# faasm/faabric

Hardware: NVIDIA H100
Metric: mpi_allreduce_resnet50_grads_algbw_GBps (higher is better)
Workload: dtype int32

## Files before the change

### csrc/kernels/coll_move_bulk.cu

```cuda
#include "coll_move.cuh"

namespace fb {

namespace {
constexpr uint32_t BULK_TILE = 32 * 1024;
constexpr int BULK_STAGES = 4;

__device__ __forceinline__ uint32_t smemPtr(const void* p)
{
    return (uint32_t)__cvta_generic_to_shared(p);
}

__device__ __forceinline__ void mbarInit(uint64_t* bar, uint32_t count)
{
    asm volatile("mbarrier.init.shared::cta.b64 [%0], %1;" ::"r"(smemPtr(bar)), "r"(count) : "memory");
}

__device__ __forceinline__ void mbarExpectTx(uint64_t* bar, uint32_t bytes)
{
    asm volatile("mbarrier.arrive.expect_tx.shared::cta.b64 _, [%0], %1;" ::"r"(smemPtr(bar)), "r"(bytes) : "memory");
}

__device__ __forceinline__ void mbarWait(uint64_t* bar, uint32_t parity)
{
    uint32_t done = 0;
    while (!done) {
        asm volatile("{\n\t"
                     ".reg .pred p;\n\t"
                     "mbarrier.try_wait.parity.shared::cta.b64 p, [%1], %2;\n\t"
                     "selp.u32 %0, 1, 0, p;\n\t"
                     "}"
                     : "=r"(done)
                     : "r"(smemPtr(bar)), "r"(parity)
                     : "memory");
    }
}

__device__ __forceinline__ void bulkLoad(void* smemDst, const void* gsrc, uint32_t bytes, uint64_t* bar)
{
    asm volatile("cp.async.bulk.shared::cluster.global.mbarrier::complete_tx::bytes [%0], [%1], %2, [%3];" ::"r"(
                   smemPtr(smemDst)),
                 "l"(gsrc),
                 "r"(bytes),
                 "r"(smemPtr(bar))
                 : "memory");
}

__device__ __forceinline__ void bulkStore(void* gdst, const void* smemSrc, uint32_t bytes)
{
    asm volatile("cp.async.bulk.global.shared::cta.bulk_group [%0], [%1], %2;" ::"l"(gdst), "r"(smemPtr(smemSrc)), "r"(bytes)
                 : "memory");
    asm volatile("cp.async.bulk.commit_group;" ::: "memory");
}

__device__ __forceinline__ void bulkWaitRead0()
{
    asm volatile("cp.async.bulk.wait_group.read 0;" ::: "memory");
}

__device__ __forceinline__ void bulkWaitAll()
{
    asm volatile("cp.async.bulk.wait_group 0;" ::: "memory");
}

__device__ __forceinline__ void fenceProxyAsync()
{
    asm volatile("fence.proxy.async;" ::: "memory");
}

struct Piece
{
    const uint8_t* src;
    uint8_t* dst;
};
}

__global__ void __launch_bounds__(128, 1) moveBulkKernel(const MoveArgs a)
{
    extern __shared__ __align__(128) uint8_t smem[];
    __shared__ __align__(8) uint64_t full[BULK_STAGES];

    BlockBarrier bar;
    bar.load(a.comm);
    bool ok = true;
    if (!a.noSync) {
        ok = bar.sync(a.comm);
    }
    const int rank = a.comm.rank;
    const int n = a.comm.nranks;

    if (threadIdx.x == 0) {
        for (int s = 0; s < BULK_STAGES; s++) {
            mbarInit(&full[s], 1);
        }
        asm volatile("fence.mbarrier_init.release.cluster;" ::: "memory");
        fenceProxyAsync();
    }
    __syncthreads();

    if (ok && threadIdx.x == 0) {
        int nPieces = 0;
        int firstPeer = 0;
        if (a.mode == MOVE_ALLGATHER || a.mode == MOVE_ALLTOALL || (a.mode == MOVE_GATHER && rank == a.root)) {
            nPieces = n;
            firstPeer = rank;
        } else if (a.mode == MOVE_SCATTER || (a.mode == MOVE_BCAST && rank != a.root)) {
            nPieces = 1;
        }
        const uint64_t srcExtra = (a.mode == MOVE_ALLTOALL) ? (uint64_t)rank * a.srcStride : 0;
        const uint64_t tilesPerPiece = (a.chunkBytes + BULK_TILE - 1) / BULK_TILE;
        const uint64_t totalTiles = (uint64_t)nPieces * tilesPerPiece;

        auto tileSrcDst = [&](uint64_t t, const uint8_t*& src, uint8_t*& dst, uint32_t& bytes) {
            const int q = (int)(t % (uint64_t)max(nPieces, 1));
            const uint64_t k = t / (uint64_t)max(nPieces, 1);
            const uint64_t off = k * BULK_TILE;
            bytes = (uint32_t)min((uint64_t)BULK_TILE, a.chunkBytes - off);
            if (a.mode == MOVE_SCATTER) {
                src = a.comm.heap[a.root] + a.sendOff + (uint64_t)rank * a.srcStride + off;
                dst = a.recvLocal + off;
            } else if (a.mode == MOVE_BCAST) {
                src = a.comm.heap[a.root] + a.sendOff + off;
                dst = a.recvLocal + off;
            } else {
                const int p = (firstPeer + q) % n;
                src = a.comm.heap[p] + a.sendOff + srcExtra + off;
                dst = a.recvLocal + (uint64_t)p * a.dstStride + off;
            }
        };

        const uint64_t first = blockIdx.x;
        const uint64_t step = gridDim.x;
        uint64_t nMine = first < totalTiles ? (totalTiles - first + step - 1) / step : 0;

        for (uint64_t j = 0; j < nMine && j < (uint64_t)BULK_STAGES; j++) {
            const uint8_t* src;
            uint8_t* dst;
            uint32_t bytes;
            tileSrcDst(first + j * step, src, dst, bytes);
            mbarExpectTx(&full[j], bytes);
            bulkLoad(smem + j * BULK_TILE, src, bytes, &full[j]);
        }
        for (uint64_t j = 0; j < nMine; j++) {
            const int s = (int)(j % BULK_STAGES);
            const uint32_t parity = (uint32_t)((j / BULK_STAGES) & 1);
            const uint8_t* src;
            uint8_t* dst;
            uint32_t bytes;
            tileSrcDst(first + j * step, src, dst, bytes);
            mbarWait(&full[s], parity);
            bulkStore(dst, smem + s * BULK_TILE, bytes);
// ... 76 lines not shown
```

### csrc/kernels/coll_reduce.cuh

```cuda
#pragma once

#include "fb_prims.cuh"
#include "launch_api.h"

namespace fb {

template<typename VR, int NR>
__device__ __forceinline__ Vec16 gatherReduce(const ReduceArgs& a,
                                              uint64_t byteOff)
{
    if constexpr (NR > 0) {
        Vec16 v[NR];
#pragma unroll
        for (int p = 0; p < NR; p++) {
            v[p] = ldVecStream(a.comm.heap[p] + a.sendOff + byteOff);
        }
        Vec16 acc = v[0];
#pragma unroll
        for (int p = 1; p < NR; p++) {
            acc = VR::apply(acc, v[p]);
        }
        return acc;
    } else {
        Vec16 acc = ldVecStream(a.comm.heap[0] + a.sendOff + byteOff);
// ... 310 lines not shown
        memcpy(&out, &v, 4);
    } else if constexpr (sizeof(E) == 8) {
        uint64_t v = *reinterpret_cast<const volatile uint64_t*>(p);
        memcpy(&out, &v, 8);
    } else {
        Vec16 v = ldVec(p);
        memcpy(&out, &v, 16);
    }
    return out;
}

template<typename E>
__device__ __forceinline__ void stElemGlobal(uint8_t* p, const E& in)
{
    if constexpr (sizeof(E) == 1) {
        uint8_t v;
        memcpy(&v, &in, 1);
        *reinterpret_cast<volatile uint8_t*>(p) = v;
    } else if constexpr (sizeof(E) == 2) {
        uint16_t v;
        memcpy(&v, &in, 2);
        *reinterpret_cast<volatile uint16_t*>(p) = v;
    } else if constexpr (sizeof(E) == 4) {
        uint32_t v;
        memcpy(&v, &in, 4);
        *reinterpret_cast<volatile uint32_t*>(p) = v;
    } else if constexpr (sizeof(E) == 8) {
        uint64_t v;
        memcpy(&v, &in, 8);
        *reinterpret_cast<volatile uint64_t*>(p) = v;
    } else {
        Vec16 v;
        memcpy(&v, &in, 16);
        stVec(p, v);
    }
}

template<typename VR>
__device__ __forceinline__ void groupTail(const FbCommDev& c,
                                          const GroupSeg& sg,
                                          int n)
{
    using Elem = typename VR::Elem;
    constexpr uint32_t EB = VR::ELEM_BYTES;
    const uint64_t base = (uint64_t)sg.nVec * 16;
    for (uint32_t e = 0; e + EB <= sg.tailBytes; e += EB) {
        Elem acc = ldElemGlobal<Elem>(c.heap[0] + sg.sendOff + base + e);
        for (int p = 1; p < n; p++) {
            Elem v = ldElemGlobal<Elem>(c.heap[p] + sg.sendOff + base + e);
            acc = VR::combine(acc, v);
        }
        for (int p = 0; p < n; p++) {
            stElemGlobal<Elem>(c.heap[p] + sg.recvOff + base + e, acc);
        }
    }
}

template<typename VR, int NR>
__global__ void __launch_bounds__(512, 1) groupAllReduceKernel(
  const GroupArgs a)
{
    extern __shared__ __align__(16) uint8_t sGroupRaw[];
    GroupSeg* sSegs = reinterpret_cast<GroupSeg*>(sGroupRaw);
    const FbCommDev& c = a.comm;
    const int n = (NR > 0) ? NR : c.nranks;
    {
        const Vec16* src = reinterpret_cast<const Vec16*>(a.segs);
        Vec16* dst = reinterpret_cast<Vec16*>(sGroupRaw);
        for (uint32_t i = threadIdx.x; i < a.nSegs * 2; i += blockDim.x) {
            dst[i] = src[i];
        }
    }
    BlockBarrier bar;
    bar.epoch = 0;
    bool ok = true;
    if (!a.noSync) {
        bar.load(c);
        ok = bar.sync(c);
    } else {
        __syncthreads();
    }

    if (ok && a.nSegs > 0) {
        constexpr int UNROLL = (NR == 8) ? 2 : (NR == 1 ? 8 : 4);
        constexpr uint32_t CHUNK = 32u * UNROLL;
        const uint32_t lane = threadIdx.x & 31;
        const uint32_t warpsPerCta = blockDim.x >> 5;
        const uint32_t warpStride = gridDim.x * warpsPerCta;
        int cur = 0;
        for (uint32_t ch = blockIdx.x * warpsPerCta + (threadIdx.x >> 5);
             ch < a.totalChunks;
             ch += warpStride) {
            if (!(sSegs[cur].chunk0 <= ch &&
                  (cur + 1 == (int)a.nSegs || ch < sSegs[cur + 1].chunk0))) {
                int lo = 0;
                int hi = (int)a.nSegs - 1;
                while (lo < hi) {
                    int mid = (lo + hi + 1) >> 1;
                    if (sSegs[mid].chunk0 <= ch) {
                        lo = mid;
                    } else {
                        hi = mid - 1;
                    }
                }
                cur = lo;
            }
            const GroupSeg sg = sSegs[cur];
            const uint32_t v0 = (ch - sg.chunk0) * CHUNK;
            const uint64_t sOff = sg.sendOff + (uint64_t)v0 * 16;
            const uint64_t rOff = sg.recvOff + (uint64_t)v0 * 16;
            const uint32_t rem = sg.nVec > v0 ? sg.nVec - v0 : 0;
            if (rem >= CHUNK) {
                Vec16 acc[UNROLL];
                if constexpr (NR > 0) {
                    Vec16 v[UNROLL][NR];
#pragma unroll
                    for (int u = 0; u < UNROLL; u++) {
#pragma unroll
                        for (int p = 0; p < NR; p++) {
                            v[u][p] = ldVecStream(c.heap[p] + sOff +
                                                  (uint64_t)(u * 32 + lane) * 16);
                        }
                    }
#pragma unroll
                    for (int u = 0; u < UNROLL; u++) {
                        acc[u] = v[u][0];
#pragma unroll
                        for (int p = 1; p < NR; p++) {
                            acc[u] = VR::apply(acc[u], v[u][p]);
                        }
                    }
#pragma unroll
                    for (int u = 0; u < UNROLL; u++) {
#pragma unroll
                        for (int p = 0; p < NR; p++) {
                            stVec(c.heap[p] + rOff + (uint64_t)(u * 32 + lane) * 16,
                                  acc[u]);
                        }
                    }
                } else {
#pragma unroll
                    for (int u = 0; u < UNROLL; u++) {
                        acc[u] = ldVecStream(c.heap[0] + sOff +
                                             (uint64_t)(u * 32 + lane) * 16);
                    }
                    for (int p = 1; p < n; p++) {
                        Vec16 v[UNROLL];
#pragma unroll
                        for (int u = 0; u < UNROLL; u++) {
                            v[u] = ldVecStream(c.heap[p] + sOff +
                                               (uint64_t)(u * 32 + lane) * 16);
                        }
#pragma unroll
                        for (int u = 0; u < UNROLL; u++) {
                            acc[u] = VR::apply(acc[u], v[u]);
                        }
                    }
                    for (int p = 0; p < n; p++) {
#pragma unroll
                        for (int u = 0; u < UNROLL; u++) {
                            stVec(c.heap[p] + rOff + (uint64_t)(u * 32 + lane) * 16,
                                  acc[u]);
                        }
                    }
                }
            } else {
#pragma unroll
                for (int u = 0; u < UNROLL; u++) {
                    const uint32_t i = (uint32_t)u * 32 + lane;
                    if (i < rem) {
                        Vec16 acc = ldVecStream(c.heap[0] + sOff + (uint64_t)i * 16);
                        for (int p = 1; p < n; p++) {
                            Vec16 v = ldVecStream(c.heap[p] + sOff + (uint64_t)i * 16);
                            acc = VR::apply(acc, v);
                        }
                        for (int p = 0; p < n; p++) {
                            stVec(c.heap[p] + rOff + (uint64_t)i * 16, acc);
                        }
                    }
                }
                if (sg.tailBytes != 0 && lane == 0 && v0 + CHUNK > sg.nVec) {
                    groupTail<VR>(c, sg, n);
                }
            }
        }
    }

    if (!a.noSync) {
        bar.sync(c);
        bar.store(c);
    }
}

template<typename VR>
cudaError_t launchGroup(const GroupArgs& a,
                        int blocks,
                        int threads,
                        cudaStream_t stream)
{
    const size_t smem = (size_t)a.nSegs * sizeof(GroupSeg);
    const int nr = a.comm.nranks;
    if (nr == 1) {
        groupAllReduceKernel<VR, 1><<<blocks, threads, smem, stream>>>(a);
    } else if (nr == 2) {
        groupAllReduceKernel<VR, 2><<<blocks, threads, smem, stream>>>(a);
    } else if (nr == 4) {
        groupAllReduceKernel<VR, 4><<<blocks, threads, smem, stream>>>(a);
    } else if (nr == 8) {
        groupAllReduceKernel<VR, 8><<<blocks, threads, smem, stream>>>(a);
    } else {
        groupAllReduceKernel<VR, 0><<<blocks, threads, smem, stream>>>(a);
    }
    return cudaGetLastError();
}

template<typename VR>
cudaError_t preloadReduce()
{
    cudaFuncAttributes a;
    cudaError_t e = cudaSuccess;
#define FB_PRELOAD(k)                                                          \
    if (e == cudaSuccess) {                                                    \
        e = cudaFuncGetAttributes(&a, k);                                      \
    }
    FB_PRELOAD((reduceKernel<VR, 0>))
    FB_PRELOAD((reduceKernel<VR, 2>))
    FB_PRELOAD((reduceKernel<VR, 4>))
    FB_PRELOAD((reduceKernel<VR, 8>))
    FB_PRELOAD((llAllReduceKernel<VR, 0>))
    FB_PRELOAD((llAllReduceKernel<VR, 2>))
    FB_PRELOAD((llAllReduceKernel<VR, 4>))
    FB_PRELOAD((llAllReduceKernel<VR, 8>))
    FB_PRELOAD((groupAllReduceKernel<VR, 0>))
    FB_PRELOAD((groupAllReduceKernel<VR, 1>))
    FB_PRELOAD((groupAllReduceKernel<VR, 2>))
    FB_PRELOAD((groupAllReduceKernel<VR, 4>))
    FB_PRELOAD((groupAllReduceKernel<VR, 8>))
#undef FB_PRELOAD
    return e;
}

template<typename VR>
const ReduceLaunchers* launchersFor()
{
    static const ReduceLaunchers l = { &launchReduce<VR>,
                                       &launchLL<VR>,
                                       &launchGroup<VR>,
                                       &preloadReduce<VR> };
    return &l;
}

}
```

### csrc/kernels/coll_reduce_pair.cu

```cuda
#include "coll_reduce.cuh"

namespace fb {

template<typename T, int OP>
static const ReduceLaunchers* LP()
{
    return launchersFor<VecReduce<T, OP, true>>();
}

template<int OP>
static const ReduceLaunchers* byPair(int dtype)
{
    switch (dtype) {
        case FB_F64_I32:
            return LP<double, OP>();
        case FB_F32_I32:
            return LP<float, OP>();
        case FB_I32_I32:
            return LP<int32_t, OP>();
        case FB_I64_I32:
            return LP<int64_t, OP>();
        default:
            return nullptr;
    }
}

const ReduceLaunchers* findReduceLaunchersPair(int dtype, int op)
{
    if (op == FB_OP_MAXLOC) {
        return byPair<FB_OP_MAXLOC>(dtype);
    }
    if (op == FB_OP_MINLOC) {
        return byPair<FB_OP_MINLOC>(dtype);
    }
    return nullptr;
}

const ReduceLaunchers* findReduceLaunchers(int dtype, int op)
{
    if (dtype >= FB_I8 && dtype <= FB_U64) {
        return findReduceLaunchersInt(dtype, op);
    }
    if (dtype >= FB_F32 && dtype <= FB_BF16) {
        return findReduceLaunchersFloat(dtype, op);
    }
    return findReduceLaunchersPair(dtype, op);
}

cudaError_t preloadAllKernels()
{
    cudaError_t e = cudaSuccess;
    for (int dt = 0; dt < FB_DTYPE_COUNT && e == cudaSuccess; dt++) {
        for (int op = 0; op < FB_OP_COUNT && e == cudaSuccess; op++) {
            const ReduceLaunchers* l = findReduceLaunchers(dt, op);
            if (l != nullptr) {
                e = l->preload();
            }
        }
    }
    if (e == cudaSuccess) {
        e = preloadMoveKernels();
    }
    if (e == cudaSuccess) {
        e = preloadMoveBulkKernel();
    }
    if (e == cudaSuccess) {
        e = preloadNvlsKernels();
    }
    if (e == cudaSuccess) {
        e = preloadStateKernels();
    }
    if (e == cudaSuccess) {
        e = preloadSnapshotKernels();
    }
    if (e == cudaSuccess) {
        e = preloadRmaKernels();
    }
    return e;
}

}
```

### csrc/kernels/launch_api.h

```cpp
#pragma once

#include <cuda_runtime.h>
#include <stdint.h>

#include "faabric/device/comm_abi.h"

namespace fb {

#define FB_NUM_SMS 132

struct ReduceArgs
{
    FbCommDev comm;
    uint64_t sendOff;
    uint64_t recvOff;
    uint8_t* recvLocal;
    uint64_t bytes;
    uint64_t vecBegin;
    uint64_t vecEnd;
    uint64_t outBase;
    int32_t readRanks;
    uint32_t pushMask;
    int32_t tailOwner;
    int32_t noSync;
};

typedef cudaError_t (*ReduceLaunchFn)(const ReduceArgs& a,
                                      int nr,
                                      int blocks,
                                      int threads,
                                      cudaStream_t stream);

#define FB_LL_BLOCKS 8
#define FB_LL_THREADS 512
#define FB_LL_MAX_VECS (FB_LL_BLOCKS * FB_LL_THREADS)
#define FB_LL_MAX_BYTES (FB_LL_MAX_VECS * 16)
#define FB_LL_AREA_BYTES(nranks) ((uint64_t)2 * (nranks) * FB_LL_MAX_VECS * 32)

struct LLArgs
{
    FbCommDev comm;
    const uint8_t* sendLocal;
    uint8_t* recvLocal;
    uint64_t bytes;
    uint64_t llOff;
    int32_t byteAccess;
    int32_t pad;
};

typedef cudaError_t (*LLLaunchFn)(const LLArgs& a, cudaStream_t stream);

struct GroupSeg
{
    uint64_t sendOff;
    uint64_t recvOff;
    uint32_t nVec;
    uint32_t chunk0;
    uint32_t tailBytes;
    uint32_t pad;
};

struct GroupArgs
{
    FbCommDev comm;
    const GroupSeg* segs;
    uint32_t nSegs;
    uint32_t totalChunks;
    int32_t noSync;
    int32_t pad;
};

static inline int fbGroupUnroll(int nranks)
{
    return (nranks == 8) ? 2 : (nranks == 1 ? 8 : 4);
}
static inline uint32_t fbGroupChunkVecs(int nranks)
{
    return 32u * (uint32_t)fbGroupUnroll(nranks);
}
#define FB_GROUP_MAX_SEGS 1024

typedef cudaError_t (*GroupLaunchFn)(const GroupArgs& a,
                                     int blocks,
                                     int threads,
                                     cudaStream_t stream);

struct ReduceLaunchers
{
    ReduceLaunchFn reduce;
    LLLaunchFn ll;
    GroupLaunchFn group;
    cudaError_t (*preload)();
};

const ReduceLaunchers* findReduceLaunchers(int dtype, int op);
const ReduceLaunchers* findReduceLaunchersInt(int dtype, int op);
const ReduceLaunchers* findReduceLaunchersFloat(int dtype, int op);
const ReduceLaunchers* findReduceLaunchersPair(int dtype, int op);


enum MoveMode
{
    MOVE_ALLGATHER = 0,
    MOVE_ALLTOALL = 1,
    MOVE_GATHER = 2,
    MOVE_SCATTER = 3,
    MOVE_BCAST = 4,
    MOVE_BCAST_2STEP = 5
};

struct MoveArgs
{
    FbCommDev comm;
    uint64_t sendOff;
    uint64_t recvOff;
    uint8_t* recvLocal;
    uint64_t chunkBytes;
    uint64_t srcStride;
    uint64_t dstStride;
    int32_t mode;
    int32_t root;
    int32_t noSync;
};

struct P2PArgs
{
    FbCommDev comm;
    uint8_t* local;
    uint64_t bytes;
    uint64_t srcOff;
    uint64_t heapBytes;
    uint64_t descOff;
    uint32_t seq;
    int32_t peer;
    int32_t stage;
    int32_t pad;
};

struct PutArgs
{
    FbCommDev comm;
    const uint8_t* local;
    uint64_t dstOff;
    uint64_t bytes;
    int32_t peer;
    int32_t signalIdx;
};

cudaError_t launchMove(const MoveArgs& a,
                       int width,
                       int blocks,
                       int threads,
                       cudaStream_t s);
cudaError_t launchBarrier(const FbCommDev& c, cudaStream_t s);
cudaError_t launchP2PSend(const P2PArgs& a, int width, int blocks, cudaStream_t s);
cudaError_t launchP2PPull(const P2PArgs& a, int width, int blocks, cudaStream_t s);
cudaError_t launchWaitWord(const FbCommDev& c,
                           const uint32_t* word,
                           uint32_t target,
                           cudaStream_t s);
cudaError_t launchSignalPeers(const FbCommDev& c,
                              uint32_t wordOff,
                              uint32_t value,
                              cudaStream_t s);
cudaError_t launchPutSignal(const PutArgs& a,
                            int width,
                            int blocks,
                            cudaStream_t s);
// ... 169 lines not shown
```

### csrc/src/device/communicator.cpp

```cpp
#include "faabric/device/communicator.h"
#include "faabric/device/nvtx.h"

#include "faabric/device/bootstrap.h"
#include "faabric/device/cuda_driver.h"
#include "launch_api.h"
#include "loopback_kernels.h"

#include <algorithm>
#include <chrono>
#include <thread>
#include <cstdio>
#include <initializer_list>
#include <barrier>
#include <cstdlib>
#include <cstring>
#include <set>
#include <shared_mutex>
#include <stdexcept>
#include <unistd.h>

namespace faabric::device {

#define CUDA_OK(expr)                                                          \
    do {                                                                       \
// ... 957 lines not shown
                freeList_[start + bytes] = rest;
            }
            allocated_[start] = bytes;
            return start;
        }
    }
    throw std::bad_alloc();
}

void Communicator::free(uint64_t offset)
{
    std::lock_guard<std::mutex> lk(allocMx_);
    auto it = allocated_.find(offset);
    if (it == allocated_.end()) {
        return;
    }
    uint64_t size = it->second;
    allocated_.erase(it);
    auto ins = freeList_.emplace(offset, size).first;
    auto next = std::next(ins);
    if (next != freeList_.end() && ins->first + ins->second == next->first) {
        ins->second += next->second;
        freeList_.erase(next);
    }
    if (ins != freeList_.begin()) {
        auto prev = std::prev(ins);
        if (prev->first + prev->second == ins->first) {
            prev->second += ins->second;
            freeList_.erase(ins);
        }
    }
}

uint8_t* Communicator::heapPtr(uint64_t offset, int rank) const
{
    if (rank < 0) {
        rank = dev_.rank;
    }
    return dev_.heap[rank] + offset;
}

bool Communicator::inHeap(const void* p, size_t bytes) const
{
    const uint8_t* b = dev_.heap[dev_.rank];
    const uint8_t* q = (const uint8_t*)p;
    return q >= b && q + bytes <= b + heapTotal_;
}

uint64_t Communicator::offsetOf(const void* p) const
{
    return (uint64_t)((const uint8_t*)p - dev_.heap[dev_.rank]);
}

namespace {
cudaError_t cudaReduce(const fb::ReduceArgs& a, int dtype, int op, int blocks, int threads, cudaStream_t s)
{
    return fb::findReduceLaunchers(dtype, op)->reduce(a, a.comm.nranks, blocks, threads, s);
}

cudaError_t cudaLL(const fb::LLArgs& a, int dtype, int op, cudaStream_t s)
{
    return fb::findReduceLaunchers(dtype, op)->ll(a, s);
}

cudaError_t cudaGroup(const fb::GroupArgs& a, int dtype, int op, int blocks, int threads, cudaStream_t s)
{
    return fb::findReduceLaunchers(dtype, op)->group(a, blocks, threads, s);
}

cudaError_t cudaCopy(void* dst, const void* src, size_t bytes, cudaStream_t s)
{
    return cudaMemcpyAsync(dst, src, bytes, cudaMemcpyDeviceToDevice, s);
}

cudaError_t cudaCopy2D(void* dst, size_t dpitch, const void* src, size_t spitch, size_t width, size_t height, cudaStream_t s)
{
    return cudaMemcpy2DAsync(dst, dpitch, src, spitch, width, height, cudaMemcpyDeviceToDevice, s);
}

const fb::KernelTable CUDA_KERNELS = {
    .reduce = cudaReduce,
    .ll = cudaLL,
    .group = cudaGroup,
    .move = fb::launchMove,
    .moveBulk = fb::launchMoveBulk,
    .barrier = fb::launchBarrier,
    .p2pSend = fb::launchP2PSend,
    .p2pPull = fb::launchP2PPull,
    .putSignal = fb::launchPutSignal,
    .waitSignal = fb::launchWaitSignal,
    .waitWord = fb::launchWaitWord,
    .signalPeers = fb::launchSignalPeers,
    .rmaAccumulate = fb::launchRmaAccumulate,
    .rmaCompareSwap = fb::launchRmaCompareSwap,
    .copy = cudaCopy,
    .copy2D = cudaCopy2D,
};

const fb::KernelTable HOST_KERNELS = {
    .reduce = fb::host::reduceKernel,
    .ll = fb::host::llAllReduce,
    .group = fb::host::groupAllReduce,
    .move = fb::host::moveKernel,
    .moveBulk = nullptr,
    .barrier = fb::host::barrierKernel,
    .p2pSend = fb::host::p2pSend,
    .p2pPull = fb::host::p2pPull,
    .putSignal = fb::host::putSignal,
    .waitSignal = fb::host::waitSignal,
    .waitWord = fb::host::waitWord,
    .signalPeers = fb::host::signalPeers,
    .rmaAccumulate = fb::host::rmaAccumulate,
    .rmaCompareSwap = fb::host::rmaCompareSwap,
    .copy = fb::host::copy,
    .copy2D = fb::host::copy2D,
};
}

int Communicator::blocksFor(uint64_t vecs, int perThread) const
{
    uint64_t perBlock = (uint64_t)cfg_.threads * perThread;
    uint64_t b = (vecs + perBlock - 1) / perBlock;
    int maxB = std::min(cfg_.maxBlocks, FB_MAX_BLOCKS / cfg_.channels);
    if (b < 1) {
        b = 1;
    }
    if (b > (uint64_t)maxB) {
        b = maxB;
    }
    return (int)b;
}

static int alignWidth(uint64_t v)
{
    if ((v & 15) == 0) {
        return 16;
    }
    if ((v & 3) == 0) {
        return 4;
    }
    return 1;
}

FbCommDev Communicator::devFor(int flags) const
{
    FbCommDev d = dev_;
    int ch = FB_FLAG_GET_CHANNEL(flags);
    if (ch >= cfg_.channels) {
        ch = ch % cfg_.channels;
    }
    d.blockBase = ch * (FB_MAX_BLOCKS / cfg_.channels);
    d.llEpochBase = ch * FB_LL_BLOCKS;
    return d;
}

void Communicator::setAllReduceTable(const std::vector<uint64_t>& maxBytes,
                                     const std::vector<int>& algos)
{
    allReduceTable_.clear();
    for (size_t i = 0; i < maxBytes.size() && i < algos.size(); i++) {
        allReduceTable_.emplace_back(maxBytes[i], algos[i]);
    }
    std::sort(allReduceTable_.begin(), allReduceTable_.end());
}

int Communicator::pickAllReduceAlgo(uint64_t bytes, bool nvlsOk) const
{
    if (!allReduceTable_.empty()) {
        int algo = allReduceTable_.back().second;
        for (const auto& [maxB, a] : allReduceTable_) {
            if (bytes <= maxB) {
                algo = a;
                break;
            }
        }
        if (algo == FB_ALGO_NVLS && !nvlsOk) {
            algo = bytes <= cfg_.oneShotMaxBytes ? FB_ALGO_ONESHOT
                                                 : FB_ALGO_TWOSHOT;
        }
        return algo;
    }
    if (bytes <= cfg_.llMaxBytes && bytes <= FB_LL_MAX_BYTES) {
        return FB_ALGO_LL;
    }
    if (nvlsOk && dev_.nranks >= 4 && bytes >= cfg_.nvlsMinBytes) {
// ... 396 lines not shown
            if (l.dSegs != nullptr) {
                cudaFree(l.dSegs);
            }
        }
        cudaGetLastError();
    }
};

struct Communicator::ManySlot
{
    fb::GroupSeg* dSegs = nullptr;
    fb::GroupSeg* hSegs = nullptr;
    cudaEvent_t ev = nullptr;
    int device = 0;
    bool used = false;
    ~ManySlot()
    {
        cudaSetDevice(device);
        if (dSegs != nullptr) {
            cudaFree(dSegs);
        }
        if (hSegs != nullptr) {
            cudaFreeHost(hSegs);
        }
        if (ev != nullptr) {
            cudaEventDestroy(ev);
        }
        cudaGetLastError();
    }
};

size_t Communicator::groupPlanLaunches(const GroupPlan& plan)
{
    return plan.launches.size();
}

namespace {
struct SegBuild
{
    std::vector<fb::GroupSeg> segs;
    uint32_t totalChunks = 0;
    uint64_t vecsPerRank = 0;
    uint64_t bytes = 0;
};
}

static int buildGroupSegs(const Communicator& c,
                          const Communicator::GroupItem* items,
                          size_t nItems,
                          size_t esize,
                          SegBuild& out)
{
    const int n = c.size();
    const int rank = c.rank();
    const uint32_t chunk = fb::fbGroupChunkVecs(n);
    uint64_t V = 0;
    for (size_t i = 0; i < nItems; i++) {
        const uint64_t bytes = (uint64_t)items[i].count * esize;
        if (bytes == 0) {
            continue;
        }
        if (!c.inHeap(items[i].send, bytes) || !c.inHeap(items[i].recv, bytes) ||
            (((uintptr_t)items[i].send | (uintptr_t)items[i].recv) & 15)) {
            return FB_E_INVALID;
        }
        V += (bytes + 15) / 16;
        out.bytes += bytes;
    }
    const uint64_t lo = V * (uint64_t)rank / n;
    const uint64_t hi = V * (uint64_t)(rank + 1) / n;
    out.vecsPerRank = (V + n - 1) / n;
    uint64_t flat = 0;
    uint64_t chunks = 0;
    for (size_t i = 0; i < nItems; i++) {
        const uint64_t bytes = (uint64_t)items[i].count * esize;
        if (bytes == 0) {
            continue;
        }
        const uint64_t vecs = (bytes + 15) / 16;
        const uint64_t full = bytes / 16;
        const uint32_t tail = (uint32_t)(bytes % 16);
        const uint64_t a = std::max(flat, lo);
        const uint64_t b = std::min(flat + vecs, hi);
        if (a < b) {
            const uint64_t v0 = a - flat;
            const uint64_t v1 = b - flat;
            fb::GroupSeg sg;
            memset(&sg, 0, sizeof(sg));
            sg.nVec = (uint32_t)(std::min(v1, full) > v0 ? std::min(v1, full) - v0 : 0);
            sg.tailBytes = (tail != 0 && v1 == vecs) ? tail : 0;
            if (sg.nVec != 0 || sg.tailBytes != 0) {
                sg.sendOff = c.offsetOf(items[i].send) + v0 * 16;
                sg.recvOff = c.offsetOf(items[i].recv) + v0 * 16;
                sg.chunk0 = (uint32_t)chunks;
                chunks += ((uint64_t)sg.nVec + (sg.tailBytes ? 1 : 0) + chunk - 1) / chunk;
                out.segs.push_back(sg);
            }
        }
        flat += vecs;
    }
    if (chunks > 0xffffffffull) {
        return FB_E_TOO_LARGE;
    }
    out.totalChunks = (uint32_t)chunks;
    return FB_OK;
}

static const size_t GROUP_ITEMS_PER_LAUNCH = FB_GROUP_MAX_SEGS - 8;

std::shared_ptr<Communicator::GroupPlan> Communicator::prepareGroup(
  const GroupItem* items,
  size_t nItems,
  int dtype,
  int* rcOut)
{
    int rcLocal = FB_OK;
    int& rc = rcOut ? *rcOut : rcLocal;
    rc = FB_OK;
    const size_t esize = fbDtypeSize(dtype);
    if (esize == 0) {
        rc = FB_E_INVALID;
        return nullptr;
    }
    bindDevice();
    auto plan = std::make_shared<GroupPlan>();
    plan->dtype = dtype;
    plan->device = device_;
    plan->items = nItems;
    for (size_t begin = 0; begin < nItems; begin += GROUP_ITEMS_PER_LAUNCH) {
        const size_t cnt = std::min(GROUP_ITEMS_PER_LAUNCH, nItems - begin);
        SegBuild sb;
        rc = buildGroupSegs(*this, items + begin, cnt, esize, sb);
        if (rc != FB_OK) {
            return nullptr;
        }
        GroupLaunch l;
        l.nSegs = (uint32_t)sb.segs.size();
        l.totalChunks = sb.totalChunks;
        l.vecsPerRank = sb.vecsPerRank;
        l.bytes = sb.bytes;
        const size_t tb = std::max<size_t>(sb.segs.size(), 1) * sizeof(fb::GroupSeg);
        if (loop_) {
            plan->hostTables = true;
            l.dSegs = (fb::GroupSeg*)::malloc(tb);
            if (!sb.segs.empty()) {
                memcpy(l.dSegs, sb.segs.data(), sb.segs.size() * sizeof(fb::GroupSeg));
            }
            plan->launches.push_back(l);
            continue;
        }
        if (cudaMalloc((void**)&l.dSegs, tb) != cudaSuccess) {
            cudaGetLastError();
            rc = FB_E_CUDA;
            return nullptr;
        }
        plan->launches.push_back(l);
        if (!sb.segs.empty() &&
            cudaMemcpy(l.dSegs, sb.segs.data(), sb.segs.size() * sizeof(fb::GroupSeg), cudaMemcpyHostToDevice) !=
              cudaSuccess) {
            cudaGetLastError();
            rc = FB_E_CUDA;
            return nullptr;
        }
    }
    return plan;
}

static int groupGrid(const CommConfig& cfg, int nranks, uint64_t vecsPerRank)
{
    const int slots = nranks == 1 ? 2 * FB_NUM_SMS : FB_MAX_BLOCKS / cfg.channels;
    const int cap = std::min(slots, cfg.groupBlocks > 0 ? cfg.groupBlocks : (nranks == 1 ? 2 * FB_NUM_SMS : 128));
    const uint64_t warps = (uint64_t)cfg.threads / 32;
    const uint64_t chunks = (vecsPerRank + fb::fbGroupChunkVecs(nranks) - 1) / fb::fbGroupChunkVecs(nranks);
    const uint64_t want = (chunks + warps * 2 - 1) / (warps * 2);
    return (int)std::clamp<uint64_t>(want, 1, (uint64_t)cap);
}

int Communicator::launchGroup(const GroupLaunch& l, int dtype, int op, int flags, cudaStream_t s)
{
    const int n = dev_.nranks;
    const bool ss = streamSync_ && !(flags & FB_FLAG_NOSYNC) && n > 1;
    fb::GroupArgs a;
    memset(&a, 0, sizeof(a));
    a.comm = devFor(flags);
    a.segs = l.dSegs;
    a.nSegs = l.nSegs;
    a.totalChunks = l.totalChunks;
    a.noSync = ((flags & FB_FLAG_NOSYNC) || ss || n == 1) ? 1 : 0;
    if (ss && streamBarrier(flags, s) != FB_OK) {
        return FB_E_CUDA;
    }
    if (k_->group(a, dtype, op, groupGrid(cfg_, n, l.vecsPerRank), cfg_.threads, s) != cudaSuccess) {
        return FB_E_CUDA;
    }
    if (ss && streamBarrier(flags, s) != FB_OK) {
        return FB_E_CUDA;
    }
    stats_.launches++;
    stats_.bytes += l.bytes;
    stats_.algoCount[FB_ALGO_TWOSHOT]++;
    return FB_OK;
}

int Communicator::allReduceGroup(const GroupPlan& plan, int op, int flags, cudaStream_t s)
{
    NvtxRange nvtxRange("fb::allReduceGroup");
    const fb::ReduceLaunchers* L = fb::findReduceLaunchers(plan.dtype, op);
    if (L == nullptr || L->group == nullptr) {
        return FB_E_UNSUPPORTED;
    }
    bindDevice();
    for (const auto& l : plan.launches) {
        int rc = launchGroup(l, plan.dtype, op, flags, s);
        if (rc != FB_OK) {
            return rc;
        }
    }
    lastAlgo_ = FB_ALGO_TWOSHOT;
    return FB_OK;
}

int Communicator::allReduceMany(const GroupItem* items,
                                size_t nItems,
                                int dtype,
                                int op,
                                int flags,
                                cudaStream_t s)
{
    NvtxRange nvtxRange("fb::allReduceMany");
    const size_t esize = fbDtypeSize(dtype);
    const fb::ReduceLaunchers* L = fb::findReduceLaunchers(dtype, op);
    if (esize == 0) {
        return FB_E_INVALID;
    }
    if (L == nullptr) {
        return FB_E_UNSUPPORTED;
    }
    bindDevice();
    for (size_t begin = 0; begin < nItems; begin += GROUP_ITEMS_PER_LAUNCH) {
        const size_t cnt = std::min(GROUP_ITEMS_PER_LAUNCH, nItems - begin);
        SegBuild sb;
        int rc = (L->group != nullptr) ? buildGroupSegs(*this, items + begin, cnt, esize, sb)
                                       : FB_E_UNSUPPORTED;
        if (rc != FB_OK) {
            for (size_t i = begin; i < begin + cnt; i++) {
                int f = flags;
                if (!inHeap(items[i].send, items[i].count * esize)) {
                    f &= ~FB_FLAG_SYMMETRIC;
                }
                int r2 = allReduce(items[i].send, items[i].recv, items[i].count, dtype, op, FB_ALGO_AUTO, f, s);
                if (r2 != FB_OK) {
                    return r2;
                }
            }
            continue;
        }
        GroupLaunch l;
        l.dSegs = sb.segs.data();
        l.nSegs = (uint32_t)sb.segs.size();
        l.totalChunks = sb.totalChunks;
        l.vecsPerRank = sb.vecsPerRank;
        l.bytes = sb.bytes;
        ManySlot* slot = nullptr;
        if (!loop_) {
            if (manySlots_.empty()) {
                manySlots_.resize(8);
            }
            auto& slotPtr = manySlots_[manyNext_++ % manySlots_.size()];
            if (!slotPtr) {
                slotPtr = std::make_shared<ManySlot>();
                slotPtr->device = device_;
                if (cudaMalloc((void**)&slotPtr->dSegs, FB_GROUP_MAX_SEGS * sizeof(fb::GroupSeg)) != cudaSuccess ||
                    cudaHostAlloc((void**)&slotPtr->hSegs, FB_GROUP_MAX_SEGS * sizeof(fb::GroupSeg), cudaHostAllocDefault) !=
                      cudaSuccess ||
                    cudaEventCreateWithFlags(&slotPtr->ev, cudaEventDisableTiming) != cudaSuccess) {
// ... 716 lines not shown
```

### csrc/src/device/loopback_kernels.cpp

```cpp
#include "loopback_kernels.h"

#include <faabric/util/reduce_ops.h>

#include <atomic>
#include <chrono>
#include <cmath>
#include <cstring>
#include <mutex>
#include <thread>

namespace fb::host {

static inline std::atomic<uint32_t>* aw(uint32_t* p)
{
    return reinterpret_cast<std::atomic<uint32_t>*>(p);
}

static inline void stRelease(uint32_t* p, uint32_t v)
{
    aw(p)->store(v, std::memory_order_release);
}

static inline uint32_t ldAcquire(const uint32_t* p)
{
// ... 358 lines not shown
            e = 1;
        }
        epochs[b] = e;
    }
    for (uint64_t i = 0; i < nVec; i++) {
        const uint32_t epoch = epochs[i / FB_LL_THREADS];
        const uint32_t par = epoch & 1;
        uint32_t w[4] = { 0, 0, 0, 0 };
        const uint64_t off = i * 16;
        const uint64_t valid = std::min<uint64_t>(16, a.bytes - off);
        memcpy(w, a.sendLocal + off, valid);
        const uint64_t slotOff = a.llOff + (((uint64_t)par * n + c.rank) * FB_LL_MAX_VECS + i) * 32;
        for (int p = 0; p < n; p++) {
            uint32_t* d = reinterpret_cast<uint32_t*>(c.heap[p] + slotOff);
            d[0] = w[0];
            d[2] = w[1];
            d[4] = w[2];
            d[6] = w[3];
            stRelease(d + 1, epoch);
            stRelease(d + 3, epoch);
            stRelease(d + 5, epoch);
            stRelease(d + 7, epoch);
        }
    }
    for (uint64_t i = 0; i < nVec && ok; i++) {
        const uint32_t epoch = epochs[i / FB_LL_THREADS];
        const uint32_t par = epoch & 1;
        uint8_t acc[16];
        for (int p = 0; p < n && ok; p++) {
            const uint32_t* s = reinterpret_cast<const uint32_t*>(
              c.heap[c.rank] + a.llOff + (((uint64_t)par * n + p) * FB_LL_MAX_VECS + i) * 32);
            for (int f = 1; f < 8 && ok; f += 2) {
                ok = waitFlagGe(c, s + f, epoch, FB_ERR_FLAG_TIMEOUT) && ldAcquire(s + f) == epoch;
            }
            uint32_t v[4] = { s[0], s[2], s[4], s[6] };
            if (p == 0) {
                memcpy(acc, v, 16);
            } else {
                for (size_t e = 0; e + es <= 16; e += es) {
                    combineElem(dtype, op, acc + e, reinterpret_cast<uint8_t*>(v) + e);
                }
            }
        }
        if (ok) {
            const uint64_t off = i * 16;
            memcpy(a.recvLocal + off, acc, std::min<uint64_t>(16, a.bytes - off));
        }
    }
    for (int b = 0; b < FB_LL_BLOCKS; b++) {
        *(c.sig[c.rank] + FB_SIG_LL_EPOCH_OFF + c.llEpochBase + b) = epochs[b];
    }
    return cudaSuccess;
}

cudaError_t groupAllReduce(const GroupArgs& a, int dtype, int op, int blocks, int, cudaStream_t)
{
    const FbCommDev& c = a.comm;
    bool ok = true;
    if (!a.noSync) {
        ok = gridBarrier(c, blocks);
    }
    if (ok) {
        const size_t es = fbDtypeSize(dtype);
        std::vector<uint8_t> tmp;
        for (uint32_t si = 0; si < a.nSegs; si++) {
            const GroupSeg& sg = a.segs[si];
            const uint64_t bytes = (uint64_t)sg.nVec * 16 + sg.tailBytes / es * es;
            if (bytes == 0) {
                continue;
            }
            tmp.resize(bytes);
            reduceRange(c, dtype, op, sg.sendOff, bytes, c.nranks, tmp.data());
            for (int p = 0; p < c.nranks; p++) {
                memcpy(c.heap[p] + sg.recvOff, tmp.data(), bytes);
            }
        }
    }
    if (!a.noSync) {
        gridBarrier(c, blocks);
    }
    return cudaSuccess;
}

cudaError_t moveKernel(const MoveArgs& a, int, int blocks, int, cudaStream_t)
{
    const FbCommDev& c = a.comm;
    const int rank = c.rank;
    const int n = c.nranks;
    bool ok = true;
    if (!a.noSync) {
        ok = gridBarrier(c, blocks);
    }
    if (ok) {
        if (a.mode == MOVE_ALLGATHER || a.mode == MOVE_ALLTOALL || (a.mode == MOVE_GATHER && rank == a.root)) {
            const uint64_t srcExtra = (a.mode == MOVE_ALLTOALL) ? (uint64_t)rank * a.srcStride : 0;
            for (int p = 0; p < n; p++) {
                memcpy(a.recvLocal + (uint64_t)p * a.dstStride, c.heap[p] + a.sendOff + srcExtra, a.chunkBytes);
            }
        } else if (a.mode == MOVE_SCATTER) {
            memcpy(a.recvLocal, c.heap[a.root] + a.sendOff + (uint64_t)rank * a.srcStride, a.chunkBytes);
        } else if (a.mode == MOVE_BCAST) {
            if (rank != a.root) {
                memcpy(a.recvLocal, c.heap[a.root] + a.sendOff, a.chunkBytes);
            }
        } else if (a.mode == MOVE_BCAST_2STEP) {
            const uint64_t total = a.chunkBytes;
            uint64_t slice = ((total / n) + 15) & ~(uint64_t)15;
            auto bounds = [&](int p, uint64_t& b, uint64_t& e) {
                b = std::min<uint64_t>((uint64_t)p * slice, total);
                e = (p == n - 1) ? total : std::min<uint64_t>(b + slice, total);
            };
            uint64_t b, e;
            bounds(rank, b, e);
            if (rank != a.root && e > b) {
                memcpy(c.heap[rank] + a.recvOff + b, c.heap[a.root] + a.sendOff + b, e - b);
            }
            ok = a.noSync ? true : gridBarrier(c, blocks);
            if (ok && rank != a.root) {
                for (int q = 1; q < n; q++) {
                    int p = (rank + q) % n;
                    bounds(p, b, e);
                    if (e <= b) {
                        continue;
                    }
                    const uint8_t* src = (p == a.root) ? c.heap[p] + a.sendOff + b : c.heap[p] + a.recvOff + b;
                    memcpy(c.heap[rank] + a.recvOff + b, src, e - b);
                }
            }
        }
    }
    if (!a.noSync) {
        gridBarrier(c, blocks);
    }
    return cudaSuccess;
}

cudaError_t barrierKernel(const FbCommDev& c, cudaStream_t)
{
    return blockBarrier(c, 0) ? cudaSuccess : cudaErrorUnknown;
}

cudaError_t p2pSend(const P2PArgs& a, int, int, cudaStream_t)
{
    const FbCommDev& c = a.comm;
    if (a.stage && a.bytes > 0) {
        memcpy(c.heap[c.rank] + a.srcOff, a.local, a.bytes);
    }
    uint32_t* desc =
      reinterpret_cast<uint32_t*>(c.heap[a.peer] + a.descOff) + ((uint32_t)c.rank * FB_P2P_RING + (a.seq % FB_P2P_RING)) * 4;
    desc[0] = (uint32_t)(a.srcOff & 0xffffffffu);
    desc[1] = (uint32_t)(a.srcOff >> 32);
    desc[2] = (uint32_t)(a.bytes & 0xffffffffu);
    desc[3] = (uint32_t)(a.bytes >> 32);
    stRelease(c.sig[a.peer] + FB_P2P_READY_OFF + c.rank, a.seq);
    return cudaSuccess;
}

cudaError_t p2pPull(const P2PArgs& a, int, int, cudaStream_t)
{
    const FbCommDev& c = a.comm;
    const uint32_t seen = ldAcquire(c.sig[c.rank] + FB_P2P_READY_OFF + a.peer);
    const uint32_t* desc = reinterpret_cast<const uint32_t*>(c.heap[c.rank] + a.descOff) +
                           ((uint32_t)a.peer * FB_P2P_RING + (a.seq % FB_P2P_RING)) * 4;
    const uint64_t srcOff = (uint64_t)desc[0] | ((uint64_t)desc[1] << 32);
    uint64_t len = (uint64_t)desc[2] | ((uint64_t)desc[3] << 32);
    if (!((int32_t)(seen - a.seq) >= 0 && len <= a.bytes && srcOff + len <= a.heapBytes)) {
// ... 159 lines not shown
```

### csrc/src/device/loopback_kernels.h

```cpp
#pragma once

#include "launch_api.h"

#include <vector>

namespace fb {

struct KernelTable
{
    cudaError_t (*reduce)(const ReduceArgs& a, int dtype, int op, int blocks, int threads, cudaStream_t s);
    cudaError_t (*ll)(const LLArgs& a, int dtype, int op, cudaStream_t s);
    cudaError_t (*group)(const GroupArgs& a, int dtype, int op, int blocks, int threads, cudaStream_t s);
    cudaError_t (*move)(const MoveArgs& a, int width, int blocks, int threads, cudaStream_t s);
    cudaError_t (*moveBulk)(const MoveArgs& a, int blocks, cudaStream_t s);
    cudaError_t (*barrier)(const FbCommDev& c, cudaStream_t s);
    cudaError_t (*p2pSend)(const P2PArgs& a, int width, int blocks, cudaStream_t s);
    cudaError_t (*p2pPull)(const P2PArgs& a, int width, int blocks, cudaStream_t s);
    cudaError_t (*putSignal)(const PutArgs& a, int width, int blocks, cudaStream_t s);
    cudaError_t (*waitSignal)(const FbCommDev& c, int signalIdx, uint32_t count, cudaStream_t s);
    cudaError_t (*waitWord)(const FbCommDev& c, const uint32_t* word, uint32_t target, cudaStream_t s);
    cudaError_t (*signalPeers)(const FbCommDev& c, uint32_t wordOff, uint32_t value, cudaStream_t s);
    cudaError_t (*rmaAccumulate)(const RmaArgs& a, int dtype, int op, cudaStream_t s);
    cudaError_t (*rmaCompareSwap)(const RmaCasArgs& a, int dtype, cudaStream_t s);
    cudaError_t (*copy)(void* dst, const void* src, size_t bytes, cudaStream_t s);
    cudaError_t (*copy2D)(void* dst,
                          size_t dpitch,
                          const void* src,
                          size_t spitch,
                          size_t width,
                          size_t height,
                          cudaStream_t s);
};

}

namespace fb::host {

bool reducible(int dtype, int op);

cudaError_t reduceKernel(const ReduceArgs& a, int dtype, int op, int blocks, int threads, cudaStream_t s);
cudaError_t llAllReduce(const LLArgs& a, int dtype, int op, cudaStream_t s);
cudaError_t groupAllReduce(const GroupArgs& a, int dtype, int op, int blocks, int threads, cudaStream_t s);
cudaError_t moveKernel(const MoveArgs& a, int width, int blocks, int threads, cudaStream_t s);
cudaError_t barrierKernel(const FbCommDev& c, cudaStream_t s);
cudaError_t p2pSend(const P2PArgs& a, int width, int blocks, cudaStream_t s);
cudaError_t p2pPull(const P2PArgs& a, int width, int blocks, cudaStream_t s);
cudaError_t putSignal(const PutArgs& a, int width, int blocks, cudaStream_t s);
cudaError_t waitSignal(const FbCommDev& c, int signalIdx, uint32_t addTarget, cudaStream_t s);
cudaError_t waitWord(const FbCommDev& c, const uint32_t* word, uint32_t target, cudaStream_t s);
cudaError_t signalPeers(const FbCommDev& c, uint32_t wordOff, uint32_t value, cudaStream_t s);
cudaError_t rmaAccumulate(const RmaArgs& a, int dtype, int op, cudaStream_t s);
cudaError_t rmaCompareSwap(const RmaCasArgs& a, int dtype, cudaStream_t s);
cudaError_t copy(void* dst, const void* src, size_t bytes, cudaStream_t s);
cudaError_t copy2D(void* dst, size_t dpitch, const void* src, size_t spitch, size_t width, size_t height, cudaStream_t s);

}
```

Baseline: 1345.

## Add dedicated single-rank group copy kernel and skip in-place segments

For single-rank communicators, grouped allreduce now launches a specialised copy kernel instead of the generic group reduce kernel. The new kernel uses 512 threads, larger 256-vector chunks per warp, streaming loads and programmatic dependent launch. Segments whose send and receive buffers are the same are dropped, since copying them is a no-op. The NR==1 instantiation of the reduce kernel is removed, and the bulk-copy helpers are moved into a shared header.

```diff
diff --git a/csrc/kernels/coll_group_copy.cu b/csrc/kernels/coll_group_copy.cu
--- /dev/null
+++ b/csrc/kernels/coll_group_copy.cu
@@ -0,0 +1,108 @@
+#include "fb_prims.cuh"
+#include "launch_api.h"
+
+namespace fb {
+
+namespace {
+
+struct CopyChunk
+{
+    const Vec16* src;
+    Vec16* dst;
+    uint32_t rem;
+    uint32_t tail;
+};
+
+__device__ __forceinline__ CopyChunk locate(const GroupSeg* segs, uint32_t nSegs, uint32_t ch, int& cur, uint8_t* heap)
+{
+    if (!(segs[cur].chunk0 <= ch && (cur + 1 == (int)nSegs || ch < segs[cur + 1].chunk0))) {
+        int lo = 0;
+        int hi = (int)nSegs - 1;
+        while (lo < hi) {
+            const int mid = (lo + hi + 1) >> 1;
+            if (segs[mid].chunk0 <= ch) {
+                lo = mid;
+            } else {
+                hi = mid - 1;
+            }
+        }
+        cur = lo;
+    }
+    constexpr uint32_t CHUNK = FB_GROUP_COPY_CHUNK_VECS;
+    const GroupSeg& sg = segs[cur];
+    const uint32_t v0 = (ch - sg.chunk0) * CHUNK;
+    CopyChunk c;
+    c.src = reinterpret_cast<const Vec16*>(heap + sg.sendOff) + v0;
+    c.dst = reinterpret_cast<Vec16*>(heap + sg.recvOff) + v0;
+    c.rem = sg.nVec > v0 ? sg.nVec - v0 : 0;
+    c.tail = (v0 + CHUNK > sg.nVec) ? sg.tailBytes : 0;
+    return c;
+}
+
+__global__ void __launch_bounds__(FB_GROUP_COPY_THREADS, FB_GROUP_COPY_CTAS_PER_SM)
+  groupCopyKernel(const GroupArgs a)
+{
+    constexpr int U = FB_GROUP_COPY_CHUNK_VECS / 32;
+    extern __shared__ __align__(16) uint8_t sCopyRaw[];
+    GroupSeg* sSegs = reinterpret_cast<GroupSeg*>(sCopyRaw);
+    asm volatile("griddepcontrol.wait;" ::: "memory");
+    {
+        const Vec16* src = reinterpret_cast<const Vec16*>(a.segs);
+        Vec16* dst = reinterpret_cast<Vec16*>(sCopyRaw);
+        for (uint32_t i = threadIdx.x; i < a.nSegs * 2; i += blockDim.x) {
+            dst[i] = src[i];
+        }
+    }
+    __syncthreads();
+
+    uint8_t* heap = a.comm.heap[0];
+    const uint32_t lane = threadIdx.x & 31;
+    const uint32_t stride = gridDim.x * (blockDim.x >> 5);
+    int cur = 0;
+    for (uint32_t ch = blockIdx.x * (blockDim.x >> 5) + (threadIdx.x >> 5); ch < a.totalChunks; ch += stride) {
+        const CopyChunk c = locate(sSegs, a.nSegs, ch, cur, heap);
+        Vec16 v[U];
+#pragma unroll
+        for (int u = 0; u < U; u++) {
+            if (u * 32 + lane < c.rem) {
+                v[u] = ldVecStream(c.src + u * 32 + lane);
+            }
+        }
+#pragma unroll
+        for (int u = 0; u < U; u++) {
+            if (u * 32 + lane < c.rem) {
+                stVec(c.dst + u * 32 + lane, v[u]);
+            }
+        }
+        if (lane < c.tail) {
+            const uint32_t t = c.rem * 16 + lane;
+            reinterpret_cast<uint8_t*>(c.dst)[t] = reinterpret_cast<const uint8_t*>(c.src)[t];
+        }
+    }
+    asm volatile("griddepcontrol.launch_dependents;" ::: "memory");
+}
+
+}
+
+cudaError_t launchGroupCopy(const GroupArgs& a, int blocks, cudaStream_t s)
+{
+    cudaLaunchConfig_t cfg = {};
+    cfg.gridDim = dim3(blocks);
+    cfg.blockDim = dim3(FB_GROUP_COPY_THREADS);
+    cfg.dynamicSmemBytes = (size_t)a.nSegs * sizeof(GroupSeg);
+    cfg.stream = s;
+    cudaLaunchAttribute attr[1];
+    attr[0].id = cudaLaunchAttributeProgrammaticStreamSerialization;
+    attr[0].val.programmaticStreamSerializationAllowed = 1;
+    cfg.attrs = attr;
+    cfg.numAttrs = 1;
+    return cudaLaunchKernelEx(&cfg, groupCopyKernel, a);
+}
+
+cudaError_t preloadGroupCopyKernel()
+{
+    cudaFuncAttributes attr;
+    return cudaFuncGetAttributes(&attr, groupCopyKernel);
+}
+
+}
diff --git a/csrc/kernels/coll_move_bulk.cu b/csrc/kernels/coll_move_bulk.cu
--- a/csrc/kernels/coll_move_bulk.cu
+++ b/csrc/kernels/coll_move_bulk.cu
@@ -1,72 +1,11 @@
 #include "coll_move.cuh"
+#include "fb_bulk.cuh"
 
 namespace fb {
 
 namespace {
 constexpr uint32_t BULK_TILE = 32 * 1024;
 constexpr int BULK_STAGES = 4;
-
-__device__ __forceinline__ uint32_t smemPtr(const void* p)
-{
-    return (uint32_t)__cvta_generic_to_shared(p);
-}
-
-__device__ __forceinline__ void mbarInit(uint64_t* bar, uint32_t count)
-{
-    asm volatile("mbarrier.init.shared::cta.b64 [%0], %1;" ::"r"(smemPtr(bar)), "r"(count) : "memory");
-}
-
-__device__ __forceinline__ void mbarExpectTx(uint64_t* bar, uint32_t bytes)
-{
-    asm volatile("mbarrier.arrive.expect_tx.shared::cta.b64 _, [%0], %1;" ::"r"(smemPtr(bar)), "r"(bytes) : "memory");
-}
-
-__device__ __forceinline__ void mbarWait(uint64_t* bar, uint32_t parity)
-{
-    uint32_t done = 0;
-    while (!done) {
-        asm volatile("{\n\t"
-                     ".reg .pred p;\n\t"
-                     "mbarrier.try_wait.parity.shared::cta.b64 p, [%1], %2;\n\t"
-                     "selp.u32 %0, 1, 0, p;\n\t"
-                     "}"
-                     : "=r"(done)
-                     : "r"(smemPtr(bar)), "r"(parity)
-                     : "memory");
-    }
-}
-
-__device__ __forceinline__ void bulkLoad(void* smemDst, const void* gsrc, uint32_t bytes, uint64_t* bar)
-{
-    asm volatile("cp.async.bulk.shared::cluster.global.mbarrier::complete_tx::bytes [%0], [%1], %2, [%3];" ::"r"(
-                   smemPtr(smemDst)),
-                 "l"(gsrc),
-                 "r"(bytes),
-                 "r"(smemPtr(bar))
-                 : "memory");
-}
-
-__device__ __forceinline__ void bulkStore(void* gdst, const void* smemSrc, uint32_t bytes)
-{
-    asm volatile("cp.async.bulk.global.shared::cta.bulk_group [%0], [%1], %2;" ::"l"(gdst), "r"(smemPtr(smemSrc)), "r"(bytes)
-                 : "memory");
-    asm volatile("cp.async.bulk.commit_group;" ::: "memory");
-}
-
-__device__ __forceinline__ void bulkWaitRead0()
-{
-    asm volatile("cp.async.bulk.wait_group.read 0;" ::: "memory");
-}
-
-__device__ __forceinline__ void bulkWaitAll()
-{
-    asm volatile("cp.async.bulk.wait_group 0;" ::: "memory");
-}
-
-__device__ __forceinline__ void fenceProxyAsync()
-{
-    asm volatile("fence.proxy.async;" ::: "memory");
-}
 
 struct Piece
 {
diff --git a/csrc/kernels/coll_reduce.cuh b/csrc/kernels/coll_reduce.cuh
--- a/csrc/kernels/coll_reduce.cuh
+++ b/csrc/kernels/coll_reduce.cuh
@@ -416,7 +416,7 @@
     }
 
     if (ok && a.nSegs > 0) {
-        constexpr int UNROLL = (NR == 8) ? 2 : (NR == 1 ? 8 : 4);
+        constexpr int UNROLL = (NR == 8) ? 2 : 4;
         constexpr uint32_t CHUNK = 32u * UNROLL;
         const uint32_t lane = threadIdx.x & 31;
         const uint32_t warpsPerCta = blockDim.x >> 5;
@@ -534,9 +534,7 @@
 {
     const size_t smem = (size_t)a.nSegs * sizeof(GroupSeg);
     const int nr = a.comm.nranks;
-    if (nr == 1) {
-        groupAllReduceKernel<VR, 1><<<blocks, threads, smem, stream>>>(a);
-    } else if (nr == 2) {
+    if (nr == 2) {
         groupAllReduceKernel<VR, 2><<<blocks, threads, smem, stream>>>(a);
     } else if (nr == 4) {
         groupAllReduceKernel<VR, 4><<<blocks, threads, smem, stream>>>(a);
@@ -566,7 +564,6 @@
     FB_PRELOAD((llAllReduceKernel<VR, 4>))
     FB_PRELOAD((llAllReduceKernel<VR, 8>))
     FB_PRELOAD((groupAllReduceKernel<VR, 0>))
-    FB_PRELOAD((groupAllReduceKernel<VR, 1>))
     FB_PRELOAD((groupAllReduceKernel<VR, 2>))
     FB_PRELOAD((groupAllReduceKernel<VR, 4>))
     FB_PRELOAD((groupAllReduceKernel<VR, 8>))
diff --git a/csrc/kernels/coll_reduce_pair.cu b/csrc/kernels/coll_reduce_pair.cu
--- a/csrc/kernels/coll_reduce_pair.cu
+++ b/csrc/kernels/coll_reduce_pair.cu
@@ -59,6 +59,9 @@
         }
     }
     if (e == cudaSuccess) {
+        e = preloadGroupCopyKernel();
+    }
+    if (e == cudaSuccess) {
         e = preloadMoveKernels();
     }
     if (e == cudaSuccess) {
diff --git a/csrc/kernels/fb_bulk.cuh b/csrc/kernels/fb_bulk.cuh
--- /dev/null
+++ b/csrc/kernels/fb_bulk.cuh
@@ -0,0 +1,69 @@
+#pragma once
+
+#include <stdint.h>
+
+namespace fb {
+
+__device__ __forceinline__ uint32_t smemPtr(const void* p)
+{
+    return (uint32_t)__cvta_generic_to_shared(p);
+}
+
+__device__ __forceinline__ void mbarInit(uint64_t* bar, uint32_t count)
+{
+    asm volatile("mbarrier.init.shared::cta.b64 [%0], %1;" ::"r"(smemPtr(bar)), "r"(count) : "memory");
+}
+
+__device__ __forceinline__ void mbarExpectTx(uint64_t* bar, uint32_t bytes)
+{
+    asm volatile("mbarrier.arrive.expect_tx.shared::cta.b64 _, [%0], %1;" ::"r"(smemPtr(bar)), "r"(bytes) : "memory");
+}
+
+__device__ __forceinline__ void mbarWait(uint64_t* bar, uint32_t parity)
+{
+    uint32_t done = 0;
+    while (!done) {
+        asm volatile("{\n\t"
+                     ".reg .pred p;\n\t"
+                     "mbarrier.try_wait.parity.shared::cta.b64 p, [%1], %2;\n\t"
+                     "selp.u32 %0, 1, 0, p;\n\t"
+                     "}"
+                     : "=r"(done)
+                     : "r"(smemPtr(bar)), "r"(parity)
+                     : "memory");
+    }
+}
+
+__device__ __forceinline__ void bulkLoad(void* smemDst, const void* gsrc, uint32_t bytes, uint64_t* bar)
+{
+    asm volatile("cp.async.bulk.shared::cluster.global.mbarrier::complete_tx::bytes [%0], [%1], %2, [%3];" ::"r"(
+                   smemPtr(smemDst)),
+                 "l"(gsrc),
+                 "r"(bytes),
+                 "r"(smemPtr(bar))
+                 : "memory");
+}
+
+__device__ __forceinline__ void bulkStore(void* gdst, const void* smemSrc, uint32_t bytes)
+{
+    asm volatile("cp.async.bulk.global.shared::cta.bulk_group [%0], [%1], %2;" ::"l"(gdst), "r"(smemPtr(smemSrc)), "r"(bytes)
+                 : "memory");
+    asm volatile("cp.async.bulk.commit_group;" ::: "memory");
+}
+
+__device__ __forceinline__ void bulkWaitRead0()
+{
+    asm volatile("cp.async.bulk.wait_group.read 0;" ::: "memory");
+}
+
+__device__ __forceinline__ void bulkWaitAll()
+{
+    asm volatile("cp.async.bulk.wait_group 0;" ::: "memory");
+}
+
+__device__ __forceinline__ void fenceProxyAsync()
+{
+    asm volatile("fence.proxy.async;" ::: "memory");
+}
+
+}
diff --git a/csrc/kernels/launch_api.h b/csrc/kernels/launch_api.h
--- a/csrc/kernels/launch_api.h
+++ b/csrc/kernels/launch_api.h
@@ -70,13 +70,14 @@
     int32_t pad;
 };
 
+#define FB_GROUP_COPY_CHUNK_VECS 256
 static inline int fbGroupUnroll(int nranks)
 {
-    return (nranks == 8) ? 2 : (nranks == 1 ? 8 : 4);
+    return (nranks == 8) ? 2 : 4;
 }
 static inline uint32_t fbGroupChunkVecs(int nranks)
 {
-    return 32u * (uint32_t)fbGroupUnroll(nranks);
+    return nranks == 1 ? FB_GROUP_COPY_CHUNK_VECS : 32u * (uint32_t)fbGroupUnroll(nranks);
 }
 #define FB_GROUP_MAX_SEGS 1024
 
@@ -84,6 +85,11 @@
                                      int blocks,
                                      int threads,
                                      cudaStream_t stream);
+
+#define FB_GROUP_COPY_THREADS 512
+#define FB_GROUP_COPY_CTAS_PER_SM 2
+cudaError_t launchGroupCopy(const GroupArgs& a, int blocks, cudaStream_t s);
+cudaError_t preloadGroupCopyKernel();
 
 struct ReduceLaunchers
 {
diff --git a/csrc/src/device/communicator.cpp b/csrc/src/device/communicator.cpp
--- a/csrc/src/device/communicator.cpp
+++ b/csrc/src/device/communicator.cpp
@@ -1063,6 +1063,7 @@
     .reduce = cudaReduce,
     .ll = cudaLL,
     .group = cudaGroup,
+    .groupCopy = fb::launchGroupCopy,
     .move = fb::launchMove,
     .moveBulk = fb::launchMoveBulk,
     .barrier = fb::launchBarrier,
@@ -1082,6 +1083,7 @@
     .reduce = fb::host::reduceKernel,
     .ll = fb::host::llAllReduce,
     .group = fb::host::groupAllReduce,
+    .groupCopy = fb::host::groupCopy,
     .move = fb::host::moveKernel,
     .moveBulk = nullptr,
     .barrier = fb::host::barrierKernel,
@@ -1644,7 +1646,7 @@
         const uint32_t tail = (uint32_t)(bytes % 16);
         const uint64_t a = std::max(flat, lo);
         const uint64_t b = std::min(flat + vecs, hi);
-        if (a < b) {
+        if (a < b && !(n == 1 && items[i].send == items[i].recv)) {
             const uint64_t v0 = a - flat;
             const uint64_t v1 = b - flat;
             fb::GroupSeg sg;
@@ -1730,12 +1732,18 @@
 
 static int groupGrid(const CommConfig& cfg, int nranks, uint64_t vecsPerRank)
 {
-    const int slots = nranks == 1 ? 2 * FB_NUM_SMS : FB_MAX_BLOCKS / cfg.channels;
-    const int cap = std::min(slots, cfg.groupBlocks > 0 ? cfg.groupBlocks : (nranks == 1 ? 2 * FB_NUM_SMS : 128));
+    const int cap = std::min(FB_MAX_BLOCKS / cfg.channels, cfg.groupBlocks > 0 ? cfg.groupBlocks : 128);
     const uint64_t warps = (uint64_t)cfg.threads / 32;
     const uint64_t chunks = (vecsPerRank + fb::fbGroupChunkVecs(nranks) - 1) / fb::fbGroupChunkVecs(nranks);
     const uint64_t want = (chunks + warps * 2 - 1) / (warps * 2);
     return (int)std::clamp<uint64_t>(want, 1, (uint64_t)cap);
+}
+
+static int groupCopyGrid(const CommConfig& cfg, uint64_t chunks)
+{
+    const uint64_t warps = FB_GROUP_COPY_THREADS / 32;
+    const uint64_t cap = cfg.groupBlocks > 0 ? (uint64_t)cfg.groupBlocks : (uint64_t)INT32_MAX;
+    return (int)std::clamp<uint64_t>((chunks + warps - 1) / warps, 1, cap);
 }
 
 int Communicator::launchGroup(const GroupLaunch& l, int dtype, int op, int flags, cudaStream_t s)
@@ -1752,7 +1760,9 @@
     if (ss && streamBarrier(flags, s) != FB_OK) {
         return FB_E_CUDA;
     }
-    if (k_->group(a, dtype, op, groupGrid(cfg_, n, l.vecsPerRank), cfg_.threads, s) != cudaSuccess) {
+    const cudaError_t e = (n == 1) ? k_->groupCopy(a, groupCopyGrid(cfg_, l.totalChunks), s)
+                                   : k_->group(a, dtype, op, groupGrid(cfg_, n, l.vecsPerRank), cfg_.threads, s);
+    if (e != cudaSuccess) {
         return FB_E_CUDA;
     }
     if (ss && streamBarrier(flags, s) != FB_OK) {
diff --git a/csrc/src/device/loopback_kernels.cpp b/csrc/src/device/loopback_kernels.cpp
--- a/csrc/src/device/loopback_kernels.cpp
+++ b/csrc/src/device/loopback_kernels.cpp
@@ -464,6 +464,16 @@
     return cudaSuccess;
 }
 
+cudaError_t groupCopy(const GroupArgs& a, int, cudaStream_t)
+{
+    uint8_t* heap = a.comm.heap[0];
+    for (uint32_t si = 0; si < a.nSegs; si++) {
+        const GroupSeg& sg = a.segs[si];
+        memcpy(heap + sg.recvOff, heap + sg.sendOff, (uint64_t)sg.nVec * 16 + sg.tailBytes);
+    }
+    return cudaSuccess;
+}
+
 cudaError_t moveKernel(const MoveArgs& a, int, int blocks, int, cudaStream_t)
 {
     const FbCommDev& c = a.comm;
diff --git a/csrc/src/device/loopback_kernels.h b/csrc/src/device/loopback_kernels.h
--- a/csrc/src/device/loopback_kernels.h
+++ b/csrc/src/device/loopback_kernels.h
@@ -11,6 +11,7 @@
     cudaError_t (*reduce)(const ReduceArgs& a, int dtype, int op, int blocks, int threads, cudaStream_t s);
     cudaError_t (*ll)(const LLArgs& a, int dtype, int op, cudaStream_t s);
     cudaError_t (*group)(const GroupArgs& a, int dtype, int op, int blocks, int threads, cudaStream_t s);
+    cudaError_t (*groupCopy)(const GroupArgs& a, int blocks, cudaStream_t s);
     cudaError_t (*move)(const MoveArgs& a, int width, int blocks, int threads, cudaStream_t s);
     cudaError_t (*moveBulk)(const MoveArgs& a, int blocks, cudaStream_t s);
     cudaError_t (*barrier)(const FbCommDev& c, cudaStream_t s);
@@ -41,6 +42,7 @@
 cudaError_t reduceKernel(const ReduceArgs& a, int dtype, int op, int blocks, int threads, cudaStream_t s);
 cudaError_t llAllReduce(const LLArgs& a, int dtype, int op, cudaStream_t s);
 cudaError_t groupAllReduce(const GroupArgs& a, int dtype, int op, int blocks, int threads, cudaStream_t s);
+cudaError_t groupCopy(const GroupArgs& a, int blocks, cudaStream_t s);
 cudaError_t moveKernel(const MoveArgs& a, int width, int blocks, int threads, cudaStream_t s);
 cudaError_t barrierKernel(const FbCommDev& c, cudaStream_t s);
 cudaError_t p2pSend(const P2PArgs& a, int width, int blocks, cudaStream_t s);
```

Measured after the change: 1406, median of 6. 4.5% higher.
